# zsc/MOSS-TTSD

Measured on AMD Instinct MI355X. Metric: audio codec tokens/sec/node (decode, bf16, batch 32 @ 4k ctx), higher is better.
Workload: dtype bf16; 1 GPU; configs[2]: batch 32 synthetic dialogues/GPU, 4k-token KV context, top-k/top-p sampling on 8 channels, decode steps at full context; batch_per_gpu=32, context=4096, prompt=512, layers=28, hidden=2048, parallelism=dp1 (batch shard, no per-step collective)

## Files before the change

### moss-ttsd_amd/csrc/attn.hip

```cpp
#include "launch.h"
#include <algorithm>
#include <atomic>
#include <cstdlib>
#ifndef MTTS_PK_WAVES
#define MTTS_PK_WAVES 0
#endif
#if MTTS_PK_WAVES
#define PK_OCC(PK) __attribute__((amdgpu_waves_per_eu((PK) ? MTTS_PK_WAVES : 1, (PK) ? MTTS_PK_WAVES : 8)))
#else
#define PK_OCC(PK)
#endif

#include "seal.h"

__device__ bool seal_lane_k(const u32x4_t* __restrict__ raw, u32x4_t* __restrict__ pk, uint8_t* __restrict__ lds, int lane) {
    u32x4_t v[16];
#pragma unroll
    for (int j = 0; j < 16; ++j) v[j] = raw[j * 64];
    __builtin_amdgcn_wave_barrier();
    uint32_t* row = (uint32_t*)(lds + lane * 128);
#pragma unroll
    for (int j = 0; j < 16; ++j)
#pragma unroll
        for (int c = 0; c < 4; c += 2) {
            const uint32_t a = u4c(v[j], c), b = u4c(v[j], c + 1);
            row[2 * j + (c >> 1)] = ((a >> 7) & 0xffu) | (((a >> 23) & 0xffu) << 8) | (((b >> 7) & 0xffu) << 16) | (((b >> 23) & 0xffu) << 24);
        }
    __builtin_amdgcn_wave_barrier();
// ... 202 lines not shown
    const float* p0 = f.partial + (size_t)r * f.Npad + col + lane;
    a = 0.f; b = 0.f;
    for (int k0 = 0; k0 < f.ksplit; k0 += 8) {
        float ta[8], tb[8];
#pragma unroll
        for (int j = 0; j < 8; ++j) {
            const float* pk = p0 + (size_t)min(k0 + j, f.ksplit - 1) * kstride;
            ta[j] = pk[0];
            tb[j] = pk[64];
        }
        if (k0 == 0) { a = ta[0]; b = tb[0]; }
#pragma unroll
        for (int j = 0; j < 8; ++j)
            if (k0 + j < f.ksplit && k0 + j > 0) { a += ta[j]; b += tb[j]; }
    }
    a = rbf(a);
    b = rbf(b);
}

__device__ __forceinline__ void fuse_reduce_request(const QkvFuse& f, int r, int col, int lane, float (&ta)[8], float (&tb)[8]) {
    const size_t kstride = (size_t)MTTS_PFCAP * f.Npad;
    const float* p0 = f.partial + (size_t)r * f.Npad + col + lane;
#pragma unroll
    for (int j = 0; j < 8; ++j) {
        const float* pk = p0 + (size_t)min(j, f.ksplit - 1) * kstride;
        ta[j] = pk[0];
        tb[j] = pk[64];
    }
}
__device__ __forceinline__ void fuse_reduce_sum(const QkvFuse& f, const float (&ta)[8], const float (&tb)[8], float& a, float& b) {
    a = ta[0]; b = tb[0];
#pragma unroll
    for (int j = 1; j < 8; ++j)
        if (j < f.ksplit) { a += ta[j]; b += tb[j]; }
    a = rbf(a);
    b = rbf(b);
}

struct FuseVec { float w0, w1, c, s; };
__device__ __forceinline__ FuseVec fuse_load_vec(const QkvFuse& f, const uint16_t* __restrict__ nw, int pos, int lane) {
    FuseVec v;
    v.w0 = bf2f(nw[lane]);
    v.w1 = bf2f(nw[lane + 64]);
    v.c = bf2f(f.rope_cos[(size_t)pos * 64 + lane]);
    v.s = bf2f(f.rope_sin[(size_t)pos * 64 + lane]);
    return v;
}
__device__ __forceinline__ void fuse_norm_rope(const QkvFuse& f, const FuseVec& v, float a, float b, float& o1, float& o2) {
    const float ss = wave_sum(a * a + b * b);
    const float inv = 1.0f / sqrtf(ss / (float)MTTS_HD + f.eps);
    a = rbf(v.w0 * rbf(a * inv));
    b = rbf(v.w1 * rbf(b * inv));
    o1 = rbf(rbf(a * v.c) + rbf(-b * v.s));
    o2 = rbf(rbf(b * v.c) + rbf(a * v.s));
}

template <int G, bool FUSED, bool PK>
__global__ __launch_bounds__(256) PK_OCC(PK) void attn_scores_kernel(
    const uint16_t* __restrict__ qbuf, u32x4_t* __restrict__ kcache, const int32_t* __restrict__ page_table,
    const RowMeta* __restrict__ meta, uint16_t* __restrict__ scores, float* __restrict__ stats, int max_pages,
    int total_pages, int nq, int nkv, float scale, QkvFuse f, const u32x4_t* __restrict__ kpack) {
    __shared__ __attribute__((aligned(16))) uint32_t qs[G][MTTS_HD / 2];
    __shared__ __attribute__((aligned(16))) uint16_t knew[MTTS_HD];
    __shared__ __attribute__((aligned(16))) uint32_t qw[PK ? 4 : 1][G][MTTS_HD / 2];
    const int r = blockIdx.z, kvh = blockIdx.y;
    const RowMeta m = meta[r];
    if (m.seq < 0) return;
    const int len = m.pos + 1;
    const int npages = (len + MTTS_PAGE - 1) / MTTS_PAGE;
// ... 367 lines not shown
#pragma unroll
        for (int j = 0; j < 8; ++j)
            if (c0 + j < nch) s += t[j];
    }
    out_packed[xpack_off(r, h * MTTS_HD + d, nq * MTTS_HD)] = f2bf(s);
}

static_assert(ROW_WAVES >= 6 && ROW_WAVES <= 16, "one wave per q head + the K row + the V row; at most 1024 threads");
static std::atomic<long long> g_row_launches{0};
long long mtts_attn_row_launches() { return g_row_launches.load(); }

template <int G, bool PK>
__global__ __launch_bounds__(ROW_WAVES * 64) void attn_row_kernel(
    u32x4_t* __restrict__ kcache, u32x4_t* __restrict__ vcache, const int32_t* __restrict__ page_table,
    const RowMeta* __restrict__ meta, uint16_t* __restrict__ out_packed, int npb, int max_pages, int total_pages, int nq,
    int nkv, float scale, QkvFuse f, const u32x4_t* __restrict__ kpack, const u32x4_t* __restrict__ vpack) {
    constexpr int W = ROW_WAVES;
    extern __shared__ __attribute__((aligned(16))) uint8_t row_lds[];
    uint32_t* qs = (uint32_t*)row_lds;
    uint16_t* knew = (uint16_t*)(row_lds + G * 256);
    uint16_t* vnew = knew + MTTS_HD;
    uint32_t* qw = (uint32_t*)(row_lds + G * 256 + 512);
    uint16_t* pbuf = (uint16_t*)((uint8_t*)qw + (PK ? W * G * 256 : 0));
    float2* st = (float2*)((uint8_t*)pbuf + W * G * 128);
    uint16_t* sc = (uint16_t*)(st + G * npb);
    float* items = (float*)(sc + (size_t)G * npb * MTTS_PAGE);
    const int r = blockIdx.y, kvh = blockIdx.x;
    const RowMeta m = meta[r];
    if (m.seq < 0) {
        for (int i = threadIdx.x; i < G * MTTS_HD; i += W * 64) out_packed[xpack_off(r, kvh * G * MTTS_HD + i, nq * MTTS_HD)] = f2bf(0.f);
        return;
    }
    const int len = m.pos + 1;
    const int npages = min((len + MTTS_PAGE - 1) / MTTS_PAGE, npb);
    const int nch = (npages + ATT_PB - 1) / ATT_PB;
    const int wave = __builtin_amdgcn_readfirstlane(threadIdx.x >> 6), lane = threadIdx.x & 63;
    const int own_pg = m.pos >> 6;
    const int sub = lane >> 5, dl = lane & 31;
    const int32_t* ptab = page_table + (size_t)m.seq * max_pages;

    const bool epi = wave < G + 2;
    const int vw = epi ? wave + W - (G + 2) : wave - (G + 2);
    if (epi) {
        const int col = (wave < G ? kvh * G + wave : wave == G ? nq + kvh : nq + nkv + kvh) * MTTS_HD;
        FuseVec pfv{0.f, 0.f, 0.f, 0.f};
        if (wave <= G) pfv = fuse_load_vec(f, wave == G ? f.knorm_w : f.qnorm_w, m.pos, lane);
        float a, b;
        if (f.ksplit <= 8) {
            float pta[8], ptb[8];
            fuse_reduce_request(f, r, col, lane, pta, ptb);
            fuse_reduce_sum(f, pta, ptb, a, b);
        } else fuse_reduce(f, r, col, lane, a, b);
        const int opage = ptab[own_pg], tok = m.pos & 63;
        if (wave <= G) {
            float o1, o2;
            fuse_norm_rope(f, pfv, a, b, o1, o2);
            if (wave < G) {
                ((uint16_t*)(qs + wave * 64))[lane] = f2bf(o1);
                ((uint16_t*)(qs + wave * 64))[lane + 64] = f2bf(o2);
            } else {
                knew[lane] = f2bf(o1);
                knew[lane + 64] = f2bf(o2);
                uint16_t* base = (uint16_t*)kcache + ((size_t)kvh * total_pages + opage) * (MTTS_PAGE * MTTS_HD);
                base[(((lane >> 3) * 64) + tok) * 8 + (lane & 7)] = f2bf(o1);
                base[((((lane + 64) >> 3) * 64) + tok) * 8 + (lane & 7)] = f2bf(o2);
            }
        } else {
            vnew[lane] = f2bf(a);
            vnew[lane + 64] = f2bf(b);
            uint16_t* dst = (uint16_t*)vcache + ((size_t)kvh * total_pages + opage) * (MTTS_PAGE * MTTS_HD) + (size_t)(tok >> 1) * (MTTS_HD * 2) + (tok & 1);
            dst[2 * lane] = f2bf(a);
            dst[2 * (lane + 64)] = f2bf(b);
        }
        __builtin_amdgcn_sched_barrier(0);
    }
    auto stage = [&]() { __syncthreads(); };

    auto finish = [&](int pg, const float* acc) {
        const int tok = pg * MTTS_PAGE + lane;
        const bool valid = tok < len;
#pragma unroll
        for (int g = 0; g < G; ++g) {
            float s = rbf(rbf(acc[g]) * scale);
            if (valid) sc[(size_t)g * npb * MTTS_PAGE + tok] = f2bf(s);
            float mx = wave_max(valid ? s : -INFINITY);
            float e = valid ? expf(s - mx) : 0.f;
            float sm = wave_sum(e);
            if (lane == 0) st[g * npb + pg] = float2{mx, sm};
        }
    };
    auto raw_dots = [&](int pg, u32x4_t (&kv)[16]) {
        if (pg == own_pg && lane == (m.pos & 63)) {
#pragma unroll
            for (int j = 0; j < 16; ++j) kv[j] = *(const u32x4_t*)&knew[8 * j];
        }
        float acc[G];
#pragma unroll
        for (int g = 0; g < G; ++g) acc[g] = 0.f;
#pragma unroll
        for (int j = 0; j < 16; ++j) {
#pragma unroll
            for (int g = 0; g < G; ++g) {
                const u32x4_t q = *(const u32x4_t*)&qs[g * 64 + 4 * j];
                acc[g] = dot2bf(kv[j].x, q.x, acc[g]);
                acc[g] = dot2bf(kv[j].y, q.y, acc[g]);
                acc[g] = dot2bf(kv[j].z, q.z, acc[g]);
                acc[g] = dot2bf(kv[j].w, q.w, acc[g]);
            }
#pragma unroll
            for (int g = 0; g < G; ++g) asm volatile("" : "+v"(acc[g]));
            if ((j & 3) == 3) __builtin_amdgcn_sched_barrier(0);
        }
        finish(pg, acc);
    };
    auto k_page = [&](int pg, bool first) {
        const int page = ptab[pg];
        const u32x4_t* kp = kcache + ((size_t)kvh * total_pages + page) * (MTTS_PAGE * MTTS_HD / 8) + lane;
        if (PK && pg < own_pg) {
            u32x4_t pk[MTTS_PKU];
            const u32x4_t* pp = kpack + ((size_t)kvh * total_pages + page) * (MTTS_PKU * 64) + lane;
#pragma unroll
            for (int j = 0; j < MTTS_PKU; ++j) pk[pk_order(j)] = __builtin_nontemporal_load(pp + pk_order(j) * 64);
            if (first) stage();
            bool qok = true;
            const uint32_t sh = pk[12].z;
            uint32_t* qwv = qw + wave * G * 64;
            __builtin_amdgcn_wave_barrier();
#pragma unroll
            for (int g = 0; g < G; ++g) {
                const uint32_t qd = qs[g * 64 + lane];
                uint32_t out = 0u;
// ... 34 lines not shown
                    acc[g] = dot2bf(w[3], q.w, acc[g]);
                }
#pragma unroll
                for (int g = 0; g < G; ++g) asm volatile("" : "+v"(acc[g]));
                if ((j & 3) == 3) __builtin_amdgcn_sched_barrier(0);
            }
            finish(pg, acc);
        } else {
            u32x4_t kv[16];
#pragma unroll
            for (int j = 0; j < 16; ++j) kv[j] = __builtin_nontemporal_load(kp + j * 64);
            if (first) stage();
            raw_dots(pg, kv);
        }
    };
    if (vw < npages) k_page(vw, true);
    else stage();
#pragma unroll 1
    for (int pg = vw + W; pg < npages; pg += W) k_page(pg, false);

    u32x4_t vv[16];
    bool packed = false;
    const u32x4_t* vp = nullptr;
    auto load_page = [&](int pg) {
        const int page = ptab[pg];
        vp = vcache + ((size_t)kvh * total_pages + page) * (MTTS_PAGE * MTTS_HD / 8) + lane;
        packed = PK && pg < own_pg;
        if (packed) {
            const u32x4_t* pp = vpack + ((size_t)kvh * total_pages + page) * (MTTS_PKU * 64) + lane;
#pragma unroll
            for (int it = 0; it < MTTS_PKU; ++it) vv[pk_order(it)] = __builtin_nontemporal_load(pp + pk_order(it) * 64);
        } else {
#pragma unroll
            for (int it = 0; it < 16; ++it) vv[it] = __builtin_nontemporal_load(vp + it * 64);
        }
    };
    if (2 * wave < npages) load_page(2 * wave);
    __syncthreads();
    float M[G], S[G];
#pragma unroll
    for (int g = 0; g < G; ++g) {
        const float2* sg = st + g * npb;
        const float2 s0 = lane < npages ? sg[lane] : float2{-INFINITY, 0.f};
        float mx = -INFINITY;
        mx = fmaxf(mx, s0.x);
        for (int p = lane + 64; p < npages; p += 64) mx = fmaxf(mx, sg[p].x);
        mx = wave_max(mx);
        float sm = 0.f;
        if (lane < npages) sm += s0.y * expf(s0.x - mx);
        for (int p = lane + 64; p < npages; p += 64) sm += sg[p].y * expf(sg[p].x - mx);
        sm = wave_sum(sm);
        M[g] = mx;
        S[g] = sm;
    }
    uint16_t* pb = pbuf + wave * G * MTTS_PAGE;
#pragma unroll 1
    for (int item = wave; item < PV_WAVES * nch; item += W) {
        float acc[G][4];
#pragma unroll
        for (int g = 0; g < G; ++g)
#pragma unroll
            for (int i = 0; i < 4; ++i) acc[g][i] = 0.f;
#pragma unroll 1
        for (int pp = 0; pp < ATT_PB / PV_WAVES; ++pp) {
            const int pg = item * (ATT_PB / PV_WAVES) + pp;
            if (pg >= npages) break;
            if (pp > 0 || item != wave) load_page(pg);
            if (pg == own_pg) {
                const int tp = (m.pos & 63) >> 1;
                if (sub == (tp & 1)) {
                    const uint32_t w01 = ((const uint32_t*)vnew)[2 * dl], w23 = ((const uint32_t*)vnew)[2 * dl + 1];
                    const uint32_t nv[4] = {w01 & 0xffffu, w01 >> 16, w23 & 0xffffu, w23 >> 16};
                    const bool hi = m.pos & 1;
#pragma unroll
                    for (int it = 0; it < 16; ++it)
                        if (it == (tp >> 1)) {
                            vv[it].x = hi ? (vv[it].x & 0xffffu) | (nv[0] << 16) : (vv[it].x & 0xffff0000u) | nv[0];
                            vv[it].y = hi ? (vv[it].y & 0xffffu) | (nv[1] << 16) : (vv[it].y & 0xffff0000u) | nv[1];
                            vv[it].z = hi ? (vv[it].z & 0xffffu) | (nv[2] << 16) : (vv[it].z & 0xffff0000u) | nv[2];
                            vv[it].w = hi ? (vv[it].w & 0xffffu) | (nv[3] << 16) : (vv[it].w & 0xffff0000u) | nv[3];
                        }
                }
            }
            uint16_t pun[G];
            bool pok = true;
            {
                const int tok = pg * MTTS_PAGE + lane;
                const int sv = (PK && packed) ? (int)(vv[12].z & 0xffu) : 0;
#pragma unroll
                for (int g = 0; g < G; ++g) {
                    float p = 0.f;
                    if (tok < len) {
                        float s = bf2f(sc[(size_t)g * npb * MTTS_PAGE + tok]);
                        p = expf(s - M[g]) / S[g];
                    }
                    uint32_t pbits = f2bf(p);
                    pun[g] = (uint16_t)pbits;
                    if (sv && (pbits & 0x7fffu)) {
                        if (((pbits >> 7) & 0xffu) == 0u) pok = false;
                        else pbits += (uint32_t)sv << 7;
                    }
                    pb[g * MTTS_PAGE + lane] = (uint16_t)pbits;
                }
            }
            __builtin_amdgcn_wave_barrier();
            if (PK && packed && __any(vv[12].w != 0u || !pok)) {
                packed = false;
#pragma unroll
                for (int it = 0; it < 16; ++it) vv[it] = __builtin_nontemporal_load(vp + it * 64);
#pragma unroll
                for (int g = 0; g < G; ++g) pb[g * MTTS_PAGE + lane] = pun[g];
// ... 34 lines not shown
            for (int i = 0; i < 4; ++i) {
                const float v = add_xor32(acc[g][i]);
                if (sub == 0) items[((size_t)item * G + g) * MTTS_HD + dl * 4 + i] = v;
            }
    }
    __syncthreads();
    for (int i = threadIdx.x; i < G * MTTS_HD; i += W * 64) {
        float s = 0.f;
        for (int c = 0; c < nch; ++c) {
            const float* it4 = items + (size_t)PV_WAVES * c * G * MTTS_HD + i;
            float v = it4[0];
#pragma unroll
            for (int w = 1; w < PV_WAVES; ++w) v += it4[(size_t)w * G * MTTS_HD];
            s += v;
        }
        out_packed[xpack_off(r, kvh * G * MTTS_HD + i, nq * MTTS_HD)] = f2bf(s);
    }
}


template <int G>
__global__ __launch_bounds__(256) void attn_prefill_scores_kernel(
    const uint16_t* __restrict__ qbuf, const u32x4_t* __restrict__ kcache, const int32_t* __restrict__ page_table,
    const RowMeta* __restrict__ meta, uint16_t* __restrict__ scores, float* __restrict__ stats, int max_pages,
    int total_pages, int nq, int nkv, float scale) {
    const int tile = blockIdx.z, kvh = blockIdx.y;
    const int wave = threadIdx.x >> 6, lane = threadIdx.x & 63;
    const int row = tile * MTTS_MAXR + (lane & 31);
    const RowMeta m0 = meta[tile * MTTS_MAXR];
    if (m0.seq < 0) return;
    const RowMeta mr = meta[row];
// ... 170 lines not shown
    }
}

static bool pv_stats_first() {
    static int v = -1;
    if (v < 0) {
        const char* g = getenv("MTTS_PV_STATS_FIRST");
        v = (g && atoi(g) == 0) ? 0 : 1;
    }
    return v != 0;
}
template <int G>
static void launch_attn_g(const void* qbuf, void* kcache, void* vcache, const int32_t* page_table,
                          const RowMeta* meta, void* scores, float* stats, float* opart, void* out_packed, int R,
                          int pages_bound, int max_pages, int total_pages, int nchunks_max, int nq, int nkv, float scale,
                          const QkvFuse* fuse, AttnPhase phase, hipStream_t st, const KvPack* pack) {
    if (phase == ATTN_PF_SCORES) {
        dim3 ga((pages_bound + 3) / 4, nkv, R / MTTS_MAXR);
        hipLaunchKernelGGL((attn_prefill_scores_kernel<G>), ga, dim3(256), 0, st, (const uint16_t*)qbuf, (const u32x4_t*)kcache,
                           page_table, meta, (uint16_t*)scores, stats, max_pages, total_pages, nq, nkv, scale);
        return;
    }
    const int nchunks_pf = (max_pages + ATT_PF - 1) / ATT_PF;
    if (phase == ATTN_PF_PV) {
        dim3 gb((pages_bound + 4 * ATT_PF - 1) / (4 * ATT_PF), nkv, R / MTTS_MAXR);
        hipLaunchKernelGGL((attn_prefill_pv_kernel<G>), gb, dim3(256), 0, st, (const uint16_t*)scores, (const float*)stats,
                           (const uint32_t*)vcache, page_table, meta, opart, max_pages, total_pages, nchunks_pf, nq, nkv);
        return;
    }
    if (phase == ATTN_PF_COMBINE) {
        hipLaunchKernelGGL(attn_combine_kernel, dim3(R, (nq + 3) / 4), dim3(512), 0, st, (const float*)opart, meta,
                           (uint16_t*)out_packed, nchunks_pf, nq, ATT_PF);
        return;
    }
    const QkvFuse f = fuse ? *fuse : QkvFuse{nullptr, 0, 0, nullptr, nullptr, nullptr, nullptr, 0.f};
    const u32x4_t* kpk = pack ? (const u32x4_t*)pack->k : nullptr;
    const u32x4_t* vpk = pack ? (const u32x4_t*)pack->v : nullptr;
    if (phase == ATTN_ROW) {
        const size_t lds = (size_t)attn_row_lds_bytes(G, kpk != nullptr, pages_bound);
        if (kpk)
            hipLaunchKernelGGL((attn_row_kernel<G, true>), dim3(nkv, R), dim3(ROW_WAVES * 64), lds, st, (u32x4_t*)kcache, (u32x4_t*)vcache,
                               page_table, meta, (uint16_t*)out_packed, pages_bound, max_pages, total_pages, nq, nkv, scale, f, kpk, vpk);
        else
            hipLaunchKernelGGL((attn_row_kernel<G, false>), dim3(nkv, R), dim3(ROW_WAVES * 64), lds, st, (u32x4_t*)kcache, (u32x4_t*)vcache,
                               page_table, meta, (uint16_t*)out_packed, pages_bound, max_pages, total_pages, nq, nkv, scale, f, kpk, vpk);
        g_row_launches.fetch_add(1);
        return;
    }
#define MTTS_SC(FU, PK)                                                                                                  \
    hipLaunchKernelGGL((attn_scores_kernel<G, FU, PK>), ga, dim3(256), 0, st, (const uint16_t*)qbuf, (u32x4_t*)kcache, \
                       page_table, meta, (uint16_t*)scores, stats, max_pages, total_pages, nq, nkv, scale, f, kpk)
#define MTTS_PV2(FU, PK, SF)                                                                                                        \
    hipLaunchKernelGGL((attn_pv_kernel<G, FU, PK, SF>), gb, dim3(PV_WAVES * 64), 0, st, (const uint16_t*)scores, (const float*)stats, \
                       (u32x4_t*)vcache, page_table, meta, opart, max_pages, total_pages, nchunks_max, nq, nkv, f, vpk)
#define MTTS_PV(FU, PK)                        \
    do {                                       \
        if (pv_stats_first()) MTTS_PV2(FU, PK, true); \
        else MTTS_PV2(FU, PK, false);          \
    } while (0)
    if (phase == ATTN_ALL || phase == ATTN_SCORES) {
// ... 34 lines not shown
        hipError_t e = hipSuccess;
#define MTTS_ROWP(GG, PK) \
    if (e == hipSuccess) e = hipFuncSetAttribute((const void*)attn_row_kernel<GG, PK>, hipFuncAttributeMaxDynamicSharedMemorySize, lim)
        MTTS_ROWP(1, false); MTTS_ROWP(1, true); MTTS_ROWP(2, false); MTTS_ROWP(2, true); MTTS_ROWP(4, false); MTTS_ROWP(4, true);
#undef MTTS_ROWP
        if (e == hipSuccess) { g_row_lds_max = lim; return 0; }
        (void)hipGetLastError();
    }
    return -1;
}
int attn_row_lds_limit() { return g_row_lds_max; }

int launch_attn(const void* qbuf, void* kcache, void* vcache, const int32_t* page_table,
                const RowMeta* meta, void* scores, float* stats, float* opart, void* out_packed, int R,
                int pages_bound, int max_pages, int total_pages, int nchunks_max, int nq, int nkv, float scale,
                const QkvFuse* fuse, AttnPhase phase, hipStream_t st, const KvPack* pack) {
    int G = nq / nkv;
    if (G != 1 && G != 2 && G != 4) return -1;
    if (phase == ATTN_ROW && !attn_row_fits(G, fuse, pack, pages_bound)) return -2;
#define MTTS_ATT(GG)                                                                                              \
    launch_attn_g<GG>(qbuf, kcache, vcache, page_table, meta, scores, stats, opart, out_packed, R, pages_bound,   \
                      max_pages, total_pages, nchunks_max, nq, nkv, scale, fuse, phase, st, pack)
    if (G == 1) MTTS_ATT(1);
    else if (G == 2) MTTS_ATT(2);
    else if (G == 4) MTTS_ATT(4);
    else return -1;
#undef MTTS_ATT
    return 0;
}
```

### moss-ttsd_amd/csrc/engine.hip

```cpp
#include "engine.h"
#include "staging.h"

#define FLUSH_STEPS 7
#define LINGER_STEPS 14
static inline int linger_bound(int B) { return 6 * B + 8; }

thread_local char g_err[512] = "";
int fail(int code, const char* fmt, ...) {
    va_list ap;
    va_start(ap, fmt);
    vsnprintf(g_err, sizeof(g_err), fmt, ap);
    va_end(ap);
    return code;
}

const char* mtts_last_error(void) { return g_err; }
int32_t mtts_version(void) { return 202; }

static auto ship_on(MttsEngine* e, hipStream_t st) {
    return [e, st](const PageEdits& ed) -> int {
        launch_set_pages(e->d_page_table, ed, st);
        HIPCHK(hipGetLastError());
        return 0;
    };
// ... 573 lines not shown
static int attend_layer(MttsEngine* e, const StepPlan& plan, int n, const RowMeta* d_meta, int R, int pages_bound, int ks_qkv,
                        hipStream_t st, int64_t kv_tokens_hint) {
    static const AttnPhase decode_ph[3] = {ATTN_SCORES, ATTN_PV, ATTN_COMBINE}, prefill_ph[3] = {ATTN_PF_SCORES, ATTN_PF_PV, ATTN_PF_COMBINE};
    Layer& l = e->layers[n];
    const AttnForm form = plan.layers[n].attn;
    const float eps = e->cfg.rms_norm_eps, scale = 1.0f / sqrtf((float)MTTS_HD);
    uint16_t* kc = (uint16_t*)e->kcache + e->layer_stride * n;
    uint16_t* vc = (uint16_t*)e->vcache + e->layer_stride * n;
    const QkvFuse fz{e->bufs.partial, ks_qkv, e->qkv_rows, (const uint16_t*)l.qn, (const uint16_t*)l.kn, e->bufs.rope_cos, e->bufs.rope_sin, eps};
    const KvPack pk = layer_pack(e, plan, n);
    const KvPack* pkp = (pk.k || pk.v) ? &pk : nullptr;
    if (form == ATTN_FORM_ROW) {
        hipEvent_t ev = nullptr;
        prof_begin(e, PROF_SCORES, st, &ev);
        if (const int rc = launch_attn(e->qbuf, kc, vc, e->d_page_table, d_meta, e->scores, e->stats, e->opart, e->attn_p, R, pages_bound,
                                       e->max_pages, e->total_pages, e->nchunks_max, e->nq, e->nkv, scale, &fz, ATTN_ROW, st, pkp))
            return fail(MTTS_EINVAL, rc == -2 ? "the whole-row attention kernel does not take this launch" : "attention group size not built");
        prof_end(e, st, ev);
        if (e->prof) e->prof_bytes[PROF_SCORES] += 2 * kv_tokens_hint * e->nkv * MTTS_HD * 2;
        return 0;
    }
    const bool fused = form == ATTN_FORM_TWO_PASS_FUSED;
    const AttnPhase* ph = form == ATTN_FORM_PREFILL_MFMA ? prefill_ph : decode_ph;
    const int nphases = plan.path == PATH_SMALL ? 2 : 3;
    if (!fused)
        launch_qkv_post(e->bufs.partial, ks_qkv, e->qkv_rows, d_meta, l.qn, l.kn, e->bufs.rope_cos, e->bufs.rope_sin, e->qbuf,
                        kc, vc, e->d_page_table, e->max_pages, e->total_pages, R, e->nq, e->nkv, eps, st);
    for (int i = 0; i < nphases; ++i) {
        hipEvent_t ev = nullptr;
        if (i < 2) prof_begin(e, i == 0 ? PROF_SCORES : PROF_PV, st, &ev);
        if (launch_attn(e->qbuf, kc, vc, e->d_page_table, d_meta, e->scores, e->stats, e->opart, e->attn_p, R,
// ... 1269 lines not shown
```

### moss-ttsd_amd/csrc/hooks.hip

```cpp
#include "engine.h"
#include "staging.h"

int32_t mtts_k_gemm_bf16(const void* w, const void* x, void* y, int32_t M, int32_t N, int32_t K, int32_t ksplit, void* stream) {
    if (!w || !x || !y || M < 1 || M > MTTS_PFCAP || K % 16 || N < 1) return fail(MTTS_EINVAL, "gemm: need 1<=M<=MTTS_PFCAP, K%%16==0");
    hipStream_t st = S(stream);
    int Npad = round_up(N, 32);
    void *wp = nullptr, *xp = nullptr;
    float* part = nullptr;
    GemmPlan p = mtts_plan_gemm(Npad, K, ksplit);
    p.depth = gemm_depth_env();
    DevBufs hb;
    TRY(hb.get((uint16_t**)&wp, (size_t)Npad * K));
    const bool tiled = M > MTTS_RCAP;
    const int ks = tiled ? (ksplit > 0 ? ksplit : mtts_tile_ksplit(Npad, K, M)) : p.ksplit;
    TRY(hb.get((uint16_t**)&xp, (size_t)MTTS_PFCAP * K));
    TRY(hb.get(&part, (size_t)ks * MTTS_PFCAP * Npad));
    launch_pack_weight(w, wp, N, K, Npad, 1, 0, st);
    const int tiles = (M + 31) / 32;
    launch_pack_rows(x, xp, M, K, tiles == 3 ? 4 : tiles, st);
    if (tiled) launch_gemm_tile(EPI_PARTIAL, M, ks, wp, xp, K, Npad, Npad, part, nullptr, st);
    else launch_gemm(EPI_PARTIAL, tiles, p, wp, xp, K, Npad, Npad, part, nullptr, st);
    launch_reduce_partial_bf16(part, y, ks, Npad, N, M, st);
    HIPCHK(hipGetLastError());
    HIPCHK(hipStreamSynchronize(st));
// ... 699 lines not shown
        HIPCHK(hipMemcpyAsync(slabs + (size_t)k * MTTS_PFCAP * Npad, dev_slabs + (size_t)k * R * Npad, (size_t)R * Npad * 4, hipMemcpyDeviceToDevice, st));
    launch_pack_kv_pages(dev_k, dev_v, kc, vc, pt, lens, R, Lmax, nkv, max_pages, total_pages, st);
    KvPack pk{nullptr, nullptr};
    if (sealed) {
        TRY(hb.get(&kp, pk_n)); TRY(hb.get(&vp, pk_n));
        launch_kv_seal_all(kc, vc, kp, vp, total_pages, nkv, 1, nullptr, st);
        pk = KvPack{kp, vp};
    }
    const QkvFuse fz{slabs, ksplit, Npad, (const uint16_t*)dev_qnw, (const uint16_t*)dev_knw, (const uint16_t*)dev_cos, (const uint16_t*)dev_sin, eps};
    const float scale = 1.0f / sqrtf((float)MTTS_HD);
    if (path == 1) {
        if (attn_row_prepare()) return fail(MTTS_EINVAL, "attn_row_kernel: the dynamic LDS limit could not be raised");
        if (!attn_row_fits(nq / nkv, &fz, sealed ? &pk : nullptr, pages_bound)) return fail(MTTS_EINVAL, "attn_section: the whole-row kernel does not take this shape");
    }
    if (const int rc = launch_attn(nullptr, kc, vc, pt, meta, scores, stats, opart, outp, MTTS_MAXR, pages_bound, max_pages, total_pages, nch,
                                   nq, nkv, scale, &fz, path == 1 ? ATTN_ROW : ATTN_ALL, st, sealed ? &pk : nullptr))
        return fail(MTTS_EINVAL, rc == -2 ? "attn_section: the whole-row kernel does not take this shape" : "attention group size not built (1, 2, 4)");
    HIPCHK(hipGetLastError());
    HIPCHK(hipMemcpyAsync(dev_out, outp, (size_t)MTTS_MAXR * nq * MTTS_HD * 2, hipMemcpyDeviceToDevice, st));
    HIPCHK(hipMemcpyAsync(dev_kcache, kc, cache_n * 2, hipMemcpyDeviceToDevice, st));
    HIPCHK(hipMemcpyAsync(dev_vcache, vc, cache_n * 2, hipMemcpyDeviceToDevice, st));
    if (sealed && dev_kpack) HIPCHK(hipMemcpyAsync(dev_kpack, kp, pk_n, hipMemcpyDeviceToDevice, st));
    if (sealed && dev_vpack) HIPCHK(hipMemcpyAsync(dev_vpack, vp, pk_n, hipMemcpyDeviceToDevice, st));
    HIPCHK(hipStreamSynchronize(st));
    return MTTS_OK;
}
int64_t mtts_debug_attn_row_launches(void) { return (int64_t)mtts_attn_row_launches(); }

int32_t mtts_k_attn_prefill(const float* dev_slabs, int32_t ksplit, const void* dev_qnw, const void* dev_knw, const void* dev_cos,
                            const void* dev_sin, float eps, const void* dev_k, const void* dev_v, const int32_t* host_lens,
                            const int32_t* host_cached, const int32_t* host_page_table, int32_t B, int32_t Lmax, int32_t nq,
// ... 138 lines not shown
                return fail(MTTS_EINVAL, "attn_bench: the whole-row kernel does not take this shape");
        }
    }
    hipEvent_t e0, e1;
    hipEventCreate(&e0); hipEventCreate(&e1);
    auto run = [&](int n) {
        for (int i = 0; i < n; ++i) {
            const int layer = i % e->L;
            uint16_t* kc = (uint16_t*)e->kcache + e->layer_stride * layer;
            uint16_t* vc = (uint16_t*)e->vcache + e->layer_stride * layer;
            const QkvFuse fz{e->bufs.partial, e->p_qkv.ksplit, e->qkv_rows, (const uint16_t*)e->layers[layer].qn,
                             (const uint16_t*)e->layers[layer].kn, e->bufs.rope_cos, e->bufs.rope_sin, e->cfg.rms_norm_eps};
            const KvPack pk = layer_pack(e, plan, layer);
            launch_attn(e->qbuf, kc, vc, e->d_page_table, e->d_meta, e->scores, e->stats, e->opart, e->attn_p, R, pages_bound,
                        e->max_pages, e->total_pages, e->nchunks_max, e->nq, e->nkv, scale, (phase == ATTN_ROW || e->B * pages_bound <= e->knobs.fuse_qkv_max) ? &fz : nullptr, (AttnPhase)phase, nullptr,
                        (pk.k || pk.v) ? &pk : nullptr);
        }
    };
    run(e->L);
    hipEventRecord(e0, nullptr);
    run(iters);
    hipEventRecord(e1, nullptr);
    HIPCHK(hipEventSynchronize(e1));
    float ms = 0;
    hipEventElapsedTime(&ms, e0, e1);
    *avg_ms = ms / iters;
    if (bytes_per_launch) {
        std::vector<RowMeta> m(MTTS_RCAP);
        HIPCHK(hipMemcpy(m.data(), e->d_meta, m.size() * sizeof(RowMeta), hipMemcpyDeviceToHost));
        int64_t tok = 0;
        for (int b = 0; b < R; ++b) if (m[b].seq >= 0) tok += m[b].pos + 1;
// ... 294 lines not shown
```

### moss-ttsd_amd/csrc/launch.h

```cpp
#pragma once
#include <type_traits>

#include "../../include/mtts.h"
#include "common.h"
#include "kvpool.h"

enum { EPI_PARTIAL = 0, EPI_BF16 = 1, EPI_SILU = 2,
       EPI_SILU_RM = 3 };
struct GemmPlan {
    int waves, ksplit, kt_per_split, kt_per_wave;
    int depth;
};
GemmPlan mtts_plan_gemm(int Npad, int K, int want_ksplit);
GemmPlan mtts_plan_gemm_forced(int Npad, int K, int ksplit, int waves);
void launch_gemm(int epi, int mb, const GemmPlan& p, const void* Wp, const void* Xp, int K, int Npad, int n_valid,
                 float* partial, uint16_t* out, hipStream_t st);
int mtts_gemm_form(int epi, int mb, const GemmPlan& p, int K, int Npad, int n_valid);
int mtts_tile_ksplit(int Npad, int K, int R);
void launch_gemm_tile(int epi, int R, int ksplit, const void* Wp, const void* Xp, int K, int Npad, int n_valid,
                      float* partial, uint16_t* out, hipStream_t st);
int mtts_small_lds_bytes(const GemmPlan& p, int K, int pro);
void launch_gemv_small(int epi, int pro, const GemmPlan& p, const void* Wp, int K, int Npad, int n_valid, float* partial,
                       uint16_t* out, const SmallPro& pr, hipStream_t st);
long long mtts_gemm_depth_launches();
// ... 28 lines not shown
void launch_set_pages(int32_t* table, const PageEdits& ed, hipStream_t st);
void launch_fork(void* kc, void* vc, size_t layer_bytes, size_t head_bytes, int blk_bytes, int L, int nkv, const ForkJob& job,
                 hipStream_t st);
void launch_pack_kv_pages(const void* K, const void* V, void* kcache, void* vcache, const int32_t* page_table, const int32_t* lens,
                          int S, int Lmax, int nkv, int max_pages, int total_pages, hipStream_t st);
void launch_bf16_to_f32(const void* a, float* b, size_t n, hipStream_t st);
void launch_unpack_rows(const void* packed, void* out, int R, int K, hipStream_t st);
void launch_bf16_round_check(unsigned long long* cnt2, hipStream_t st);

enum AttnPhase { ATTN_ALL = 0, ATTN_SCORES = 1, ATTN_PV = 2, ATTN_COMBINE = 3,
                 ATTN_ROW = 4,
                 ATTN_PF_SCORES = 11, ATTN_PF_PV = 12, ATTN_PF_COMBINE = 13 };
int launch_attn(const void* qbuf, void* kcache, void* vcache, const int32_t* page_table,
                const RowMeta* meta, void* scores, float* stats, float* opart, void* out_packed, int R,
                int pages_bound, int max_pages, int total_pages, int nchunks_max, int nq, int nkv, float scale,
                const QkvFuse* fuse, AttnPhase phase, hipStream_t st, const KvPack* pack = nullptr);
bool attn_row_fits(int G, const QkvFuse* fuse, const KvPack* pack, int pages_bound);
int attn_row_prepare();
int attn_row_lds_limit();
long long mtts_attn_row_launches();
void launch_kv_seal_rows(const void* kcache, const void* vcache, void* kpack, void* vpack, const int32_t* page_table,
                         const RowMeta* meta, int R, int max_pages, int total_pages, int nkv, int L, unsigned long long* cnt, hipStream_t st);
void launch_kv_seal_all(const void* kcache, const void* vcache, void* kpack, void* vpack, int total_pages, int nkv, int L,
                        unsigned long long* cnt, hipStream_t st);
void launch_kv_seal_pages(const void* raw, void* pk, int npages, int as_k, hipStream_t st);
void launch_kv_pack_count(const void* kpack, const void* vpack, const int32_t* page_table, const int32_t* complete, int B, int max_pages,
                          int total_pages, int nkv, int L, unsigned long long* out, hipStream_t st);

struct SeqState {
    int32_t nas;
    int32_t unfinished;
// ... 145 lines not shown
```

### moss-ttsd_amd/csrc/shapes.h

```cpp
#pragma once
#include <stdint.h>

#define MTTS_MAXR 32
#define MTTS_RCAP 128
#define MTTS_PFCAP 2048
#define MTTS_PAGE 64
#define ATT_PB 8
#define ATT_PF 2
#define SMALL_RP 4

struct RowMeta {
    int32_t seq;
    int32_t pos;
    int32_t last;
    int32_t pad;
};

#define BIAS_RULES 64
#define BIAS_RULE_LEN 16
struct BiasRules {
    int32_t n;
    int32_t len[BIAS_RULES];
    float beta[BIAS_RULES];
    int32_t ids[BIAS_RULES][BIAS_RULE_LEN];
// ... 1 lines not shown

enum { WSEAL_GU = 0, WSEAL_DOWN = 1, WSEAL_HEAD0 = 2, WSEAL_HEADS = 3, WSEAL_KINDS = 4 };

enum { GEMM_SKINNY = 0, GEMM_DEPTH = 1, GEMM_GATEUP48 = 2 };

#ifndef PV_WAVES
#define PV_WAVES 4
#endif
#ifndef ROW_WAVES
#define ROW_WAVES 12
#endif
static inline int attn_row_lds_bytes(int G, bool pk, int pages_bound) {
    const int nch = (pages_bound + ATT_PB - 1) / ATT_PB;
    return G * 256 + 512 + (pk ? ROW_WAVES * G * 256 : 0) + ROW_WAVES * G * 128 + G * pages_bound * (8 + 128) + PV_WAVES * nch * G * 512;
}
```

### moss-ttsd_amd/csrc/stepplan.h

```cpp
#pragma once
#include <algorithm>
#include <cstdio>
#include <cstdlib>
#include <string>
#include <vector>

#include "shapes.h"

#define MTTS_FOLD_NORM_DEFAULT 0
struct StepKnobs {
    int small_rows = SMALL_RP;
    int fuse_qkv_max = 2560;
    int pack_min_work = 512;
    int attn_row = 1;
    int pf_mfma_pages = 0;
    int gemm_depth = 1;
    int fold_norm = MTTS_FOLD_NORM_DEFAULT;
    int w_seal = 1;
    int w_seal_head = 1;
    int kv_pack = 1;
    bool use_graphs = true;
};
static inline StepKnobs step_knobs_from_env() {
    StepKnobs k;
    const auto clamp = [](const char* g, int lo, int hi) { return std::min(std::max(atoi(g), lo), hi); };
    if (const char* g = getenv("MTTS_GRAPHS")) k.use_graphs = atoi(g) != 0;
    if (const char* g = getenv("MTTS_FUSE_QKV_MAX")) k.fuse_qkv_max = atoi(g);
    if (const char* g = getenv("MTTS_KV_PACK")) k.kv_pack = atoi(g);
    if (const char* g = getenv("MTTS_KV_PACK_MIN")) k.pack_min_work = atoi(g);
    if (const char* g = getenv("MTTS_PREFILL_MFMA_PAGES")) k.pf_mfma_pages = atoi(g);
    if (const char* g = getenv("MTTS_ATTN_ROW")) k.attn_row = clamp(g, 0, 2);
    if (const char* g = getenv("MTTS_SMALL_ROWS")) k.small_rows = clamp(g, 0, SMALL_RP);
    if (const char* g = getenv("MTTS_GEMM_DEPTH")) k.gemm_depth = atoi(g) != 0;
    if (const char* g = getenv("MTTS_FOLD_NORM")) k.fold_norm = atoi(g) != 0;
    if (const char* g = getenv("MTTS_W_SEAL")) k.w_seal = clamp(g, 0, 2);
    if (const char* g = getenv("MTTS_W_SEAL_HEAD")) k.w_seal_head = atoi(g) != 0;
    return k;
}
static inline int fold_norm_env() { return step_knobs_from_env().fold_norm; }
static inline int gemm_depth_env() { return step_knobs_from_env().gemm_depth; }

enum { GEMM_QKV = 0, GEMM_O = 1, GEMM_GU = 2, GEMM_DOWN = 3, GEMM_HEAD0 = 4, GEMM_HEADS = 5,
       GEMM_GU_SLAB = 6,
       GEMM_KINDS = 7 };
struct StepCaps {
    int G = 1, nkv = 1, L = 0;
    int n_cus = 0;
    bool f32 = false;
    bool small_fits = false;
    bool fold_shape = false;
    int row_lds_limit = 0;
    bool wseal_kind[WSEAL_KINDS] = {false, false, false, false};
    int gemm_form[GEMM_KINDS] = {0, 0, 0, 0, 0, 0, 0};
};

// ... 140 lines not shown
```

Before: 83720 codec_tokens/s.

## Prefetch page ids and fused-QKV partials before meta load in row attention

The whole-row attention kernel now issues its page-table reads and the split-K QKV partial loads before reading the row metadata. It speculatively assumes row r maps to sequence r and keeps the page ids in registers, reading them with readlane. It falls back to the page table when the assumption fails. Separately, bf16 rounding is done with paired pack2_rn conversions in norm/rope, the score scaling, the softmax probabilities and the output store. The aim is to hide the dependent global-load latency at kernel start and cut conversion instructions, at the cost of extra registers, more complex code and a new default-on knob.

After: 84360 codec_tokens/s, median of 6. Within noise of the previous version (+0.8%).

```diff
diff --git a/moss-ttsd_amd/csrc/attn.hip b/moss-ttsd_amd/csrc/attn.hip
--- a/moss-ttsd_amd/csrc/attn.hip
+++ b/moss-ttsd_amd/csrc/attn.hip
@@ -12,6 +12,7 @@
 #endif
 
 #include "seal.h"
+#include "norm_ops.h"
 
 __device__ bool seal_lane_k(const u32x4_t* __restrict__ raw, u32x4_t* __restrict__ pk, uint8_t* __restrict__ lds, int lane) {
     u32x4_t v[16];
@@ -244,8 +245,9 @@
         for (int j = 0; j < 8; ++j)
             if (k0 + j < f.ksplit && k0 + j > 0) { a += ta[j]; b += tb[j]; }
     }
-    a = rbf(a);
-    b = rbf(b);
+    const uint32_t ab = pack2_rn(a, b);
+    a = bflo(ab);
+    b = bfhi(ab);
 }
 
 __device__ __forceinline__ void fuse_reduce_request(const QkvFuse& f, int r, int col, int lane, float (&ta)[8], float (&tb)[8]) {
@@ -263,26 +265,49 @@
 #pragma unroll
     for (int j = 1; j < 8; ++j)
         if (j < f.ksplit) { a += ta[j]; b += tb[j]; }
-    a = rbf(a);
-    b = rbf(b);
+    const uint32_t ab = pack2_rn(a, b);
+    a = bflo(ab);
+    b = bfhi(ab);
 }
 
 struct FuseVec { float w0, w1, c, s; };
+__device__ __forceinline__ void fuse_load_w(FuseVec& v, const uint16_t* __restrict__ nw, int lane) {
+    v.w0 = bf2f(nw[lane]);
+    v.w1 = bf2f(nw[lane + 64]);
+}
+__device__ __forceinline__ void fuse_load_w_raw(uint32_t (&w)[2], const uint16_t* __restrict__ nw, int lane) {
+    w[0] = nw[lane];
+    w[1] = nw[lane + 64];
+}
+__device__ __forceinline__ void fuse_take_w(FuseVec& v, uint32_t (&w)[2]) {
+    asm volatile("" : "+v"(w[0]), "+v"(w[1]));
+    v.w0 = __uint_as_float(w[0] << 16);
+    v.w1 = __uint_as_float(w[1] << 16);
+}
+__device__ __forceinline__ void fuse_load_rope(FuseVec& v, const QkvFuse& f, int pos, int lane) {
+    v.c = bf2f(f.rope_cos[(size_t)pos * 64 + lane]);
+    v.s = bf2f(f.rope_sin[(size_t)pos * 64 + lane]);
+}
 __device__ __forceinline__ FuseVec fuse_load_vec(const QkvFuse& f, const uint16_t* __restrict__ nw, int pos, int lane) {
     FuseVec v;
-    v.w0 = bf2f(nw[lane]);
-    v.w1 = bf2f(nw[lane + 64]);
-    v.c = bf2f(f.rope_cos[(size_t)pos * 64 + lane]);
-    v.s = bf2f(f.rope_sin[(size_t)pos * 64 + lane]);
+    fuse_load_w(v, nw, lane);
+    fuse_load_rope(v, f, pos, lane);
     return v;
 }
-__device__ __forceinline__ void fuse_norm_rope(const QkvFuse& f, const FuseVec& v, float a, float b, float& o1, float& o2) {
+__device__ __forceinline__ uint32_t fuse_norm_rope2(const QkvFuse& f, const FuseVec& v, float a, float b) {
     const float ss = wave_sum(a * a + b * b);
     const float inv = 1.0f / sqrtf(ss / (float)MTTS_HD + f.eps);
-    a = rbf(v.w0 * rbf(a * inv));
-    b = rbf(v.w1 * rbf(b * inv));
-    o1 = rbf(rbf(a * v.c) + rbf(-b * v.s));
-    o2 = rbf(rbf(b * v.c) + rbf(a * v.s));
+    uint32_t t = pack2_rn(a * inv, b * inv);
+    t = pack2_rn(v.w0 * bflo(t), v.w1 * bfhi(t));
+    a = bflo(t);
+    b = bfhi(t);
+    const uint32_t x = pack2_rn(a * v.c, -b * v.s), y = pack2_rn(b * v.c, a * v.s);
+    return pack2_rn(bflo(x) + bfhi(x), bflo(y) + bfhi(y));
+}
+__device__ __forceinline__ void fuse_norm_rope(const QkvFuse& f, const FuseVec& v, float a, float b, float& o1, float& o2) {
+    const uint32_t o = fuse_norm_rope2(f, v, a, b);
+    o1 = bflo(o);
+    o2 = bfhi(o);
 }
 
 template <int G, bool FUSED, bool PK>
@@ -680,7 +705,7 @@
 __global__ __launch_bounds__(ROW_WAVES * 64) void attn_row_kernel(
     u32x4_t* __restrict__ kcache, u32x4_t* __restrict__ vcache, const int32_t* __restrict__ page_table,
     const RowMeta* __restrict__ meta, uint16_t* __restrict__ out_packed, int npb, int max_pages, int total_pages, int nq,
-    int nkv, float scale, QkvFuse f, const u32x4_t* __restrict__ kpack, const u32x4_t* __restrict__ vpack) {
+    int nkv, float scale, QkvFuse f, const u32x4_t* __restrict__ kpack, const u32x4_t* __restrict__ vpack, int table_rows) {
     constexpr int W = ROW_WAVES;
     extern __shared__ __attribute__((aligned(16))) uint8_t row_lds[];
     uint32_t* qs = (uint32_t*)row_lds;
@@ -692,7 +717,29 @@
     uint16_t* sc = (uint16_t*)(st + G * npb);
     float* items = (float*)(sc + (size_t)G * npb * MTTS_PAGE);
     const int r = blockIdx.y, kvh = blockIdx.x;
+    const int wave = __builtin_amdgcn_readfirstlane(threadIdx.x >> 6), lane = threadIdx.x & 63;
+    const bool epi = wave < G + 2;
+    const int vw = epi ? wave + W - (G + 2) : wave - (G + 2);
+    const int ecol = (wave < G ? kvh * G + wave : wave == G ? nq + kvh : nq + nkv + kvh) * MTTS_HD;
+    const uint16_t* enw = wave == G ? f.knorm_w : f.qnorm_w;
+
     const RowMeta m = meta[r];
+    const bool early = table_rows > 0;
+    const bool pre = early && epi && f.ksplit <= 8;
+    int kid = 0, vid = 0;
+    float pta[8], ptb[8];
+    FuseVec pfv{0.f, 0.f, 0.f, 0.f};
+    uint32_t pw[2] = {0u, 0u};
+    if (early) {
+        const int32_t* trow = page_table + (size_t)min(r, table_rows - 1) * max_pages;
+        const int lastp = min(npb, max_pages) - 1;
+        kid = trow[min(vw + W * lane, lastp)];
+        vid = trow[min(2 * (wave + W * (lane >> 1)) + (lane & 1), lastp)];
+    }
+    if (pre) {
+        fuse_reduce_request(f, r, ecol, lane, pta, ptb);
+        if (wave <= G) fuse_load_w_raw(pw, enw, lane);
+    }
     if (m.seq < 0) {
         for (int i = threadIdx.x; i < G * MTTS_HD; i += W * 64) out_packed[xpack_off(r, kvh * G * MTTS_HD + i, nq * MTTS_HD)] = f2bf(0.f);
         return;
@@ -700,43 +747,45 @@
     const int len = m.pos + 1;
     const int npages = min((len + MTTS_PAGE - 1) / MTTS_PAGE, npb);
     const int nch = (npages + ATT_PB - 1) / ATT_PB;
-    const int wave = __builtin_amdgcn_readfirstlane(threadIdx.x >> 6), lane = threadIdx.x & 63;
     const int own_pg = m.pos >> 6;
     const int sub = lane >> 5, dl = lane & 31;
     const int32_t* ptab = page_table + (size_t)m.seq * max_pages;
-
-    const bool epi = wave < G + 2;
-    const int vw = epi ? wave + W - (G + 2) : wave - (G + 2);
+    const bool fast = early && m.seq == r;
+
     if (epi) {
-        const int col = (wave < G ? kvh * G + wave : wave == G ? nq + kvh : nq + nkv + kvh) * MTTS_HD;
-        FuseVec pfv{0.f, 0.f, 0.f, 0.f};
-        if (wave <= G) pfv = fuse_load_vec(f, wave == G ? f.knorm_w : f.qnorm_w, m.pos, lane);
+        const int opage = ptab[own_pg], tok = m.pos & 63;
         float a, b;
-        if (f.ksplit <= 8) {
-            float pta[8], ptb[8];
-            fuse_reduce_request(f, r, col, lane, pta, ptb);
+        if (pre) {
+            if (wave <= G) fuse_load_rope(pfv, f, m.pos, lane);
+            fuse_take_w(pfv, pw);
             fuse_reduce_sum(f, pta, ptb, a, b);
-        } else fuse_reduce(f, r, col, lane, a, b);
-        const int opage = ptab[own_pg], tok = m.pos & 63;
+        } else {
+            if (wave <= G) pfv = fuse_load_vec(f, enw, m.pos, lane);
+            if (f.ksplit <= 8) {
+                fuse_reduce_request(f, r, ecol, lane, pta, ptb);
+                fuse_reduce_sum(f, pta, ptb, a, b);
+            } else fuse_reduce(f, r, ecol, lane, a, b);
+        }
         if (wave <= G) {
-            float o1, o2;
-            fuse_norm_rope(f, pfv, a, b, o1, o2);
+            const uint32_t o = fuse_norm_rope2(f, pfv, a, b);
+            const uint16_t o1 = (uint16_t)o, o2 = (uint16_t)(o >> 16);
             if (wave < G) {
-                ((uint16_t*)(qs + wave * 64))[lane] = f2bf(o1);
-                ((uint16_t*)(qs + wave * 64))[lane + 64] = f2bf(o2);
+                ((uint16_t*)(qs + wave * 64))[lane] = o1;
+                ((uint16_t*)(qs + wave * 64))[lane + 64] = o2;
             } else {
-                knew[lane] = f2bf(o1);
-                knew[lane + 64] = f2bf(o2);
+                knew[lane] = o1;
+                knew[lane + 64] = o2;
                 uint16_t* base = (uint16_t*)kcache + ((size_t)kvh * total_pages + opage) * (MTTS_PAGE * MTTS_HD);
-                base[(((lane >> 3) * 64) + tok) * 8 + (lane & 7)] = f2bf(o1);
-                base[((((lane + 64) >> 3) * 64) + tok) * 8 + (lane & 7)] = f2bf(o2);
+                base[(((lane >> 3) * 64) + tok) * 8 + (lane & 7)] = o1;
+                base[((((lane + 64) >> 3) * 64) + tok) * 8 + (lane & 7)] = o2;
             }
         } else {
-            vnew[lane] = f2bf(a);
-            vnew[lane + 64] = f2bf(b);
+            const uint16_t v1 = (uint16_t)(__float_as_uint(a) >> 16), v2 = (uint16_t)(__float_as_uint(b) >> 16);
+            vnew[lane] = v1;
+            vnew[lane + 64] = v2;
             uint16_t* dst = (uint16_t*)vcache + ((size_t)kvh * total_pages + opage) * (MTTS_PAGE * MTTS_HD) + (size_t)(tok >> 1) * (MTTS_HD * 2) + (tok & 1);
-            dst[2 * lane] = f2bf(a);
-            dst[2 * (lane + 64)] = f2bf(b);
+            dst[2 * lane] = v1;
+            dst[2 * (lane + 64)] = v2;
         }
         __builtin_amdgcn_sched_barrier(0);
     }
@@ -745,10 +794,16 @@
     auto finish = [&](int pg, const float* acc) {
         const int tok = pg * MTTS_PAGE + lane;
         const bool valid = tok < len;
+        uint32_t sb[(G + 1) / 2];
+#pragma unroll
+        for (int g = 0; g < G; g += 2) {
+            const uint32_t d = pack2_rn(acc[g], g + 1 < G ? acc[g + 1] : 0.f);
+            sb[g / 2] = pack2_rn(bflo(d) * scale, bfhi(d) * scale);
+        }
 #pragma unroll
         for (int g = 0; g < G; ++g) {
-            float s = rbf(rbf(acc[g]) * scale);
-            if (valid) sc[(size_t)g * npb * MTTS_PAGE + tok] = f2bf(s);
+            const float s = (g & 1) ? bfhi(sb[g / 2]) : bflo(sb[g / 2]);
+            if (valid) sc[(size_t)g * npb * MTTS_PAGE + tok] = (uint16_t)(sb[g / 2] >> (16 * (g & 1)));
             float mx = wave_max(valid ? s : -INFINITY);
             float e = valid ? expf(s - mx) : 0.f;
             float sm = wave_sum(e);
@@ -779,8 +834,8 @@
         }
         finish(pg, acc);
     };
-    auto k_page = [&](int pg, bool first) {
-        const int page = ptab[pg];
+    auto k_page = [&](int pg, int k, bool first) {
+        const int page = fast ? __builtin_amdgcn_readlane(kid, k) : ptab[pg];
         const u32x4_t* kp = kcache + ((size_t)kvh * total_pages + page) * (MTTS_PAGE * MTTS_HD / 8) + lane;
         if (PK && pg < own_pg) {
             u32x4_t pk[MTTS_PKU];
@@ -845,16 +900,17 @@
             raw_dots(pg, kv);
         }
     };
-    if (vw < npages) k_page(vw, true);
+    if (vw < npages) k_page(vw, 0, true);
     else stage();
 #pragma unroll 1
-    for (int pg = vw + W; pg < npages; pg += W) k_page(pg, false);
+    for (int pg = vw + W, k = 1; pg < npages; pg += W, ++k) k_page(pg, k, false);
 
     u32x4_t vv[16];
     bool packed = false;
     const u32x4_t* vp = nullptr;
-    auto load_page = [&](int pg) {
-        const int page = ptab[pg];
+    static_assert(ATT_PB / PV_WAVES == 2, "vid holds two page ids per work item");
+    auto load_page = [&](int pg, int idl) {
+        const int page = fast ? __builtin_amdgcn_readlane(vid, idl) : ptab[pg];
         vp = vcache + ((size_t)kvh * total_pages + page) * (MTTS_PAGE * MTTS_HD / 8) + lane;
         packed = PK && pg < own_pg;
         if (packed) {
@@ -866,7 +922,7 @@
             for (int it = 0; it < 16; ++it) vv[it] = __builtin_nontemporal_load(vp + it * 64);
         }
     };
-    if (2 * wave < npages) load_page(2 * wave);
+    if (2 * wave < npages) load_page(2 * wave, 0);
     __syncthreads();
     float M[G], S[G];
 #pragma unroll
@@ -886,7 +942,7 @@
     }
     uint16_t* pb = pbuf + wave * G * MTTS_PAGE;
 #pragma unroll 1
-    for (int item = wave; item < PV_WAVES * nch; item += W) {
+    for (int item = wave, j = 0; item < PV_WAVES * nch; item += W, ++j) {
         float acc[G][4];
 #pragma unroll
         for (int g = 0; g < G; ++g)
@@ -896,7 +952,7 @@
         for (int pp = 0; pp < ATT_PB / PV_WAVES; ++pp) {
             const int pg = item * (ATT_PB / PV_WAVES) + pp;
             if (pg >= npages) break;
-            if (pp > 0 || item != wave) load_page(pg);
+            if (pp > 0 || item != wave) load_page(pg, 2 * j + pp);
             if (pg == own_pg) {
                 const int tp = (m.pos & 63) >> 1;
                 if (sub == (tp & 1)) {
@@ -918,14 +974,20 @@
             {
                 const int tok = pg * MTTS_PAGE + lane;
                 const int sv = (PK && packed) ? (int)(vv[12].z & 0xffu) : 0;
+                float pf[G + 1];
 #pragma unroll
                 for (int g = 0; g < G; ++g) {
-                    float p = 0.f;
+                    pf[g] = 0.f;
                     if (tok < len) {
                         float s = bf2f(sc[(size_t)g * npb * MTTS_PAGE + tok]);
-                        p = expf(s - M[g]) / S[g];
+                        pf[g] = expf(s - M[g]) / S[g];
                     }
-                    uint32_t pbits = f2bf(p);
+                }
+                pf[G] = 0.f;
+#pragma unroll
+                for (int g = 0; g < G; ++g) {
+                    const uint32_t p2 = pack2_rn(pf[g & ~1], pf[(g & ~1) + 1]);
+                    uint32_t pbits = (g & 1) ? p2 >> 16 : p2 & 0xffffu;
                     pun[g] = (uint16_t)pbits;
                     if (sv && (pbits & 0x7fffu)) {
                         if (((pbits >> 7) & 0xffu) == 0u) pok = false;
@@ -990,7 +1052,7 @@
             for (int w = 1; w < PV_WAVES; ++w) v += it4[(size_t)w * G * MTTS_HD];
             s += v;
         }
-        out_packed[xpack_off(r, kvh * G * MTTS_HD + i, nq * MTTS_HD)] = f2bf(s);
+        out_packed[xpack_off(r, kvh * G * MTTS_HD + i, nq * MTTS_HD)] = (uint16_t)pack2_rn(s, 0.f);
     }
 }
 
@@ -1191,7 +1253,7 @@
 static void launch_attn_g(const void* qbuf, void* kcache, void* vcache, const int32_t* page_table,
                           const RowMeta* meta, void* scores, float* stats, float* opart, void* out_packed, int R,
                           int pages_bound, int max_pages, int total_pages, int nchunks_max, int nq, int nkv, float scale,
-                          const QkvFuse* fuse, AttnPhase phase, hipStream_t st, const KvPack* pack) {
+                          const QkvFuse* fuse, AttnPhase phase, hipStream_t st, const KvPack* pack, int table_rows) {
     if (phase == ATTN_PF_SCORES) {
         dim3 ga((pages_bound + 3) / 4, nkv, R / MTTS_MAXR);
         hipLaunchKernelGGL((attn_prefill_scores_kernel<G>), ga, dim3(256), 0, st, (const uint16_t*)qbuf, (const u32x4_t*)kcache,
@@ -1215,12 +1277,13 @@
     const u32x4_t* vpk = pack ? (const u32x4_t*)pack->v : nullptr;
     if (phase == ATTN_ROW) {
         const size_t lds = (size_t)attn_row_lds_bytes(G, kpk != nullptr, pages_bound);
+        const int trows = pages_bound <= ATTN_ROW_ID_PAGES ? std::max(table_rows, 0) : 0;
         if (kpk)
             hipLaunchKernelGGL((attn_row_kernel<G, true>), dim3(nkv, R), dim3(ROW_WAVES * 64), lds, st, (u32x4_t*)kcache, (u32x4_t*)vcache,
-                               page_table, meta, (uint16_t*)out_packed, pages_bound, max_pages, total_pages, nq, nkv, scale, f, kpk, vpk);
+                               page_table, meta, (uint16_t*)out_packed, pages_bound, max_pages, total_pages, nq, nkv, scale, f, kpk, vpk, trows);
         else
             hipLaunchKernelGGL((attn_row_kernel<G, false>), dim3(nkv, R), dim3(ROW_WAVES * 64), lds, st, (u32x4_t*)kcache, (u32x4_t*)vcache,
-                               page_table, meta, (uint16_t*)out_packed, pages_bound, max_pages, total_pages, nq, nkv, scale, f, kpk, vpk);
+                               page_table, meta, (uint16_t*)out_packed, pages_bound, max_pages, total_pages, nq, nkv, scale, f, kpk, vpk, trows);
         g_row_launches.fetch_add(1);
         return;
     }
@@ -1285,13 +1348,13 @@
 int launch_attn(const void* qbuf, void* kcache, void* vcache, const int32_t* page_table,
                 const RowMeta* meta, void* scores, float* stats, float* opart, void* out_packed, int R,
                 int pages_bound, int max_pages, int total_pages, int nchunks_max, int nq, int nkv, float scale,
-                const QkvFuse* fuse, AttnPhase phase, hipStream_t st, const KvPack* pack) {
+                const QkvFuse* fuse, AttnPhase phase, hipStream_t st, const KvPack* pack, int table_rows) {
     int G = nq / nkv;
     if (G != 1 && G != 2 && G != 4) return -1;
     if (phase == ATTN_ROW && !attn_row_fits(G, fuse, pack, pages_bound)) return -2;
 #define MTTS_ATT(GG)                                                                                              \
     launch_attn_g<GG>(qbuf, kcache, vcache, page_table, meta, scores, stats, opart, out_packed, R, pages_bound,   \
-                      max_pages, total_pages, nchunks_max, nq, nkv, scale, fuse, phase, st, pack)
+                      max_pages, total_pages, nchunks_max, nq, nkv, scale, fuse, phase, st, pack, table_rows)
     if (G == 1) MTTS_ATT(1);
     else if (G == 2) MTTS_ATT(2);
     else if (G == 4) MTTS_ATT(4);
diff --git a/moss-ttsd_amd/csrc/engine.hip b/moss-ttsd_amd/csrc/engine.hip
--- a/moss-ttsd_amd/csrc/engine.hip
+++ b/moss-ttsd_amd/csrc/engine.hip
@@ -611,7 +611,8 @@
         hipEvent_t ev = nullptr;
         prof_begin(e, PROF_SCORES, st, &ev);
         if (const int rc = launch_attn(e->qbuf, kc, vc, e->d_page_table, d_meta, e->scores, e->stats, e->opart, e->attn_p, R, pages_bound,
-                                       e->max_pages, e->total_pages, e->nchunks_max, e->nq, e->nkv, scale, &fz, ATTN_ROW, st, pkp))
+                                       e->max_pages, e->total_pages, e->nchunks_max, e->nq, e->nkv, scale, &fz, ATTN_ROW, st, pkp,
+                                       e->knobs.attn_row_start ? e->cfg.max_batch : 0))
             return fail(MTTS_EINVAL, rc == -2 ? "the whole-row attention kernel does not take this launch" : "attention group size not built");
         prof_end(e, st, ev);
         if (e->prof) e->prof_bytes[PROF_SCORES] += 2 * kv_tokens_hint * e->nkv * MTTS_HD * 2;
diff --git a/moss-ttsd_amd/csrc/hooks.hip b/moss-ttsd_amd/csrc/hooks.hip
--- a/moss-ttsd_amd/csrc/hooks.hip
+++ b/moss-ttsd_amd/csrc/hooks.hip
@@ -737,7 +737,7 @@
         if (!attn_row_fits(nq / nkv, &fz, sealed ? &pk : nullptr, pages_bound)) return fail(MTTS_EINVAL, "attn_section: the whole-row kernel does not take this shape");
     }
     if (const int rc = launch_attn(nullptr, kc, vc, pt, meta, scores, stats, opart, outp, MTTS_MAXR, pages_bound, max_pages, total_pages, nch,
-                                   nq, nkv, scale, &fz, path == 1 ? ATTN_ROW : ATTN_ALL, st, sealed ? &pk : nullptr))
+                                   nq, nkv, scale, &fz, path == 1 ? ATTN_ROW : ATTN_ALL, st, sealed ? &pk : nullptr, attn_row_start_env() ? R : 0))
         return fail(MTTS_EINVAL, rc == -2 ? "attn_section: the whole-row kernel does not take this shape" : "attention group size not built (1, 2, 4)");
     HIPCHK(hipGetLastError());
     HIPCHK(hipMemcpyAsync(dev_out, outp, (size_t)MTTS_MAXR * nq * MTTS_HD * 2, hipMemcpyDeviceToDevice, st));
@@ -906,7 +906,7 @@
             const KvPack pk = layer_pack(e, plan, layer);
             launch_attn(e->qbuf, kc, vc, e->d_page_table, e->d_meta, e->scores, e->stats, e->opart, e->attn_p, R, pages_bound,
                         e->max_pages, e->total_pages, e->nchunks_max, e->nq, e->nkv, scale, (phase == ATTN_ROW || e->B * pages_bound <= e->knobs.fuse_qkv_max) ? &fz : nullptr, (AttnPhase)phase, nullptr,
-                        (pk.k || pk.v) ? &pk : nullptr);
+                        (pk.k || pk.v) ? &pk : nullptr, e->knobs.attn_row_start ? e->cfg.max_batch : 0);
         }
     };
     run(e->L);
diff --git a/moss-ttsd_amd/csrc/launch.h b/moss-ttsd_amd/csrc/launch.h
--- a/moss-ttsd_amd/csrc/launch.h
+++ b/moss-ttsd_amd/csrc/launch.h
@@ -66,7 +66,7 @@
 int launch_attn(const void* qbuf, void* kcache, void* vcache, const int32_t* page_table,
                 const RowMeta* meta, void* scores, float* stats, float* opart, void* out_packed, int R,
                 int pages_bound, int max_pages, int total_pages, int nchunks_max, int nq, int nkv, float scale,
-                const QkvFuse* fuse, AttnPhase phase, hipStream_t st, const KvPack* pack = nullptr);
+                const QkvFuse* fuse, AttnPhase phase, hipStream_t st, const KvPack* pack = nullptr, int table_rows = 0);
 bool attn_row_fits(int G, const QkvFuse* fuse, const KvPack* pack, int pages_bound);
 int attn_row_prepare();
 int attn_row_lds_limit();
diff --git a/moss-ttsd_amd/csrc/shapes.h b/moss-ttsd_amd/csrc/shapes.h
--- a/moss-ttsd_amd/csrc/shapes.h
+++ b/moss-ttsd_amd/csrc/shapes.h
@@ -39,3 +39,4 @@
     const int nch = (pages_bound + ATT_PB - 1) / ATT_PB;
     return G * 256 + 512 + (pk ? ROW_WAVES * G * 256 : 0) + ROW_WAVES * G * 128 + G * pages_bound * (8 + 128) + PV_WAVES * nch * G * 512;
 }
+#define ATTN_ROW_ID_PAGES (64 * ROW_WAVES)
diff --git a/moss-ttsd_amd/csrc/stepplan.h b/moss-ttsd_amd/csrc/stepplan.h
--- a/moss-ttsd_amd/csrc/stepplan.h
+++ b/moss-ttsd_amd/csrc/stepplan.h
@@ -13,6 +13,7 @@
     int fuse_qkv_max = 2560;
     int pack_min_work = 512;
     int attn_row = 1;
+    int attn_row_start = 1;
     int pf_mfma_pages = 0;
     int gemm_depth = 1;
     int fold_norm = MTTS_FOLD_NORM_DEFAULT;
@@ -30,6 +31,7 @@
     if (const char* g = getenv("MTTS_KV_PACK_MIN")) k.pack_min_work = atoi(g);
     if (const char* g = getenv("MTTS_PREFILL_MFMA_PAGES")) k.pf_mfma_pages = atoi(g);
     if (const char* g = getenv("MTTS_ATTN_ROW")) k.attn_row = clamp(g, 0, 2);
+    if (const char* g = getenv("MTTS_ATTN_ROW_START")) k.attn_row_start = atoi(g) != 0;
     if (const char* g = getenv("MTTS_SMALL_ROWS")) k.small_rows = clamp(g, 0, SMALL_RP);
     if (const char* g = getenv("MTTS_GEMM_DEPTH")) k.gemm_depth = atoi(g) != 0;
     if (const char* g = getenv("MTTS_FOLD_NORM")) k.fold_norm = atoi(g) != 0;
@@ -39,6 +41,7 @@
 }
 static inline int fold_norm_env() { return step_knobs_from_env().fold_norm; }
 static inline int gemm_depth_env() { return step_knobs_from_env().gemm_depth; }
+static inline int attn_row_start_env() { return step_knobs_from_env().attn_row_start; }
 
 enum { GEMM_QKV = 0, GEMM_O = 1, GEMM_GU = 2, GEMM_DOWN = 3, GEMM_HEAD0 = 4, GEMM_HEADS = 5,
        GEMM_GU_SLAB = 6,
```
